# proger/haloop

Measured on AMD Instinct MI355X. Metric: utterances/sec, LSTM-CTC training step (fwd + CTC loss + bwd + clip + AdamW), higher is better.
Workload: dtype bf16 (dense operands rounded to bf16, 1 MFMA per product, fp32 accumulate; fp32 state, CTC, optimizer and master weights); 1 GPU; LC-2x1024: conv(80->128,k5,s4) + 2-layer LSTM H=1024 + Linear(1024->32) + CTC, 80 frames x 80 mels, vocab 32, targets 5-10 symbols, dropout 0.2; batch_per_gpu=64, global_batch=64, frames=80, mels=80, parallelism=dp1, hip_graph=False, math=bf16

## Files before the change

haloop_amd/csrc/lstm.hip:

```cpp
#include <stdlib.h>
#include <string.h>
#include "halo_common.h"
#include "halo_internal.h"
#include "tiled_image.h"
#include "lstm_persist.h"

namespace {

enum YMode { Y_NONE = 0, Y_PLAIN = 1, Y_RELU = 2, Y_DROPOUT = 3 };

typedef __bf16 bf16x8 __attribute__((ext_vector_type(8)));

template <bool X3>
struct Packed {
    static constexpr int KB = X3 ? 32 : 16;
    static constexpr int BLOCK_BYTES = X3 ? 2048 : 1024;
    __device__ static __forceinline__ void store(void *img, int tile, int nk, int i, int k, float v) {
        const int blk = k / KB, kk = k % KB;
        char *base = (char *)img + ((long)tile * (nk / KB) + blk) * BLOCK_BYTES;
        if (X3) {
            const int lane = (kk >> 3) * 16 + i, e = kk & 7;
            const __bf16 hi = (__bf16)v;
            const __bf16 lo = (__bf16)(v - (float)hi);
            reinterpret_cast<__bf16 *>(base)[lane * 8 + e] = hi;
// ... 437 lines not shown
        else if (u < a.w_units + a.s_units) pack_unit<true, 2>(u - a.w_units, a.h0, a.hp0, a.H, a.B, a.H, a.h_rm, a.c0, a.c_rm);
        else if (u < a.w_units + a.s_units + a.zero_units) reinterpret_cast<uint4 *>(a.zero)[u - a.w_units - a.s_units] = make_uint4(0u, 0u, 0u, 0u);
        else reinterpret_cast<uint4 *>(a.zero2)[u - a.w_units - a.s_units - a.zero_units] = make_uint4(0u, 0u, 0u, 0u);
    }
}

struct ImageJobs {
    struct { const float *src; int R, K, ld, KT, tr, first; char *img; } job[4];
    int n, blocks, with_lo;
};
__device__ __forceinline__ void image_jobs_block(const ImageJobs &a, int b, float *tile) {
    int j = 0;
#pragma unroll
    for (int i = 1; i < 4; ++i)
        if (i < a.n && b >= a.job[i].first) j = i;
    const int local = b - a.job[j].first, kt = local % a.job[j].KT, rt = local / a.job[j].KT;
    if (a.job[j].tr)
        halo_img::prep_transposed_block(a.job[j].src, a.job[j].R, a.job[j].K, a.job[j].ld, a.job[j].img, a.job[j].KT, a.with_lo, kt, rt,
                                        reinterpret_cast<float (*)[halo_img::TR + 1]>(tile));
    else
        halo_img::prep_rowmajor_block(a.job[j].src, a.job[j].R, a.job[j].K, a.job[j].ld, a.job[j].img, a.job[j].KT, a.with_lo, kt, rt);
}
inline void image_jobs_add(ImageJobs &a, const float *src, int R, int K, int ld, int tr, char *img) {
    const int KT = (K + 31) / 32;
    a.job[a.n++] = {src, R, K, ld, KT, tr, a.blocks, img};
    a.blocks += ((R + 127) / 128) * KT;
}

struct Prologue2Args {
    const float *w[3]; void *wdst[3]; long w_units; int wK;
    const float *h0[2]; void *hp0[2]; float *h_rm[2]; const float *c0[2]; float *c_rm[2]; long s_units;
    unsigned *zero; long zero_units;
    unsigned *zero2; long zero2_units;
    char *arm[3]; int narm; long arm_units;
    int H, B;
    ImageJobs img;
};
__device__ __forceinline__ void arm_unit(const Prologue2Args &a, long v) {
    const int m = (int)(v / a.arm_units);
    const long w = v - m * a.arm_units;
    *reinterpret_cast<uint4 *>(a.arm[m] + (w >> 6) * 2048 + (w & 63) * 16) = make_uint4(~0u, ~0u, ~0u, ~0u);
}
template <int WMODE>
__global__ __launch_bounds__(256) void persist2_prologue_kernel(const Prologue2Args a) {
    if ((int)blockIdx.x < a.img.blocks) {
        __shared__ float tile[32 * (halo_img::TR + 1)];
        image_jobs_block(a.img, blockIdx.x, tile);
        return;
    }
    const long nw = 3 * a.w_units, ns = 2 * a.s_units, na = (long)a.narm * a.arm_units;
    const long total = nw + ns + a.zero_units + a.zero2_units + na;
    for (long u = (blockIdx.x - a.img.blocks) * 256L + threadIdx.x; u < total; u += (long)(gridDim.x - a.img.blocks) * 256) {
        if (u >= total - na) {
            arm_unit(a, u - (total - na));
        } else if (u < nw) {
            const int m = (int)(u / a.w_units);
            pack_unit<true, WMODE, true>(u - m * a.w_units, a.w[m], a.wdst[m], a.H, a.B, a.wK, nullptr, nullptr, nullptr);
        } else if (u < nw + ns) {
            const int l = (int)((u - nw) / a.s_units);
            pack_unit<true, 2, true>(u - nw - l * a.s_units, a.h0[l], a.hp0[l], a.H, a.B, a.H, a.h_rm[l], a.c0[l], a.c_rm[l]);
        } else if (u < nw + ns + a.zero_units) {
            reinterpret_cast<uint4 *>(a.zero)[u - nw - ns] = make_uint4(0u, 0u, 0u, 0u);
        } else {
            reinterpret_cast<uint4 *>(a.zero2)[u - nw - ns - a.zero_units] = make_uint4(0u, 0u, 0u, 0u);
        }
    }
}
// ... 788 lines not shown
        if (images_by_pack)
            HALO_TRY(halo_gemm_bf16x3_tiled(img_in, img_w, T * B, 4 * H, in_dim, l0.gates, 4 * H, b_ih[0], b_hh[0], 0, nullptr, st));
        ctx.packF_stamp = lo == 0 ? ctx.lstm_weights_stamp : 0;
        ctx.packF_reserve = reserve;
        for (int m = 0; m < 3; ++m) ctx.packF_w[m] = pa.w[m];
        memcpy(ctx.packF_dims, dims, sizeof(dims));
    }
    Persist2Fwd a;
    a.wp0 = (const char *)wp0; a.wp1 = (const char *)wp1; a.wpi = (const char *)wpi;
    a.hp0 = (char *)l0.hp; a.hp1 = (char *)l1.hp;
    a.xp = xp;
    a.gates0 = l0.gates; a.h0 = l0.h; a.c0 = l0.c;
    a.gates1 = l1.gates; a.h1 = l1.h; a.c1 = l1.c;
    a.b_ih1 = b_ih[1]; a.b_hh1 = b_hh[1];
    a.ydrop = p_drop > 0.f ? l0.ydrop : nullptr;
    a.y = y; a.y_stride_t = y_stride_t; a.y_stride_b = y_stride_b; a.y_mode = y ? (y_relu ? 2 : 1) : 0;
    a.drop = make_dropout(p_drop, seed, HALO_STREAM_LSTM_LAYER0 + (uint32_t)lo, offset, offset_dev);
    a.img_hT0 = emit_hT0; a.img_hT1 = emit_hT1; a.img_xT1 = emit_xT1;
    a.flags = flags;
    a.stamps = halo_lstm_persist_stamp_buffer();
    a.T = T; a.B = B; a.H = H;
    chain_begin(st);
    HALO_TRY(halo_lstm_persist2_fwd(a, st));
    chain_end(st, 0, 1, "lstm_persist2_fwd_kernel");
    for (int l = 0; l < 2; ++l) {
        const LayerBufs lb = l ? l1 : l0;
        if (hn) HALO_TRY(copy_d2d(hn + (size_t)(lo + l) * BH, lb.h + (size_t)T * BH, BH, st));
        if (cn) HALO_TRY(copy_d2d(cn + (size_t)(lo + l) * BH, lb.c + (size_t)T * BH, BH, st));
    }
    return HALO_OK;
}


inline size_t bwd_p2_offset(int T, int B, int in0, int H, int L) {
    const size_t n = bwd_flags_offset(T, B, in0, H, L) + PERSIST_FLAG_BYTES + (size_t)((B + 15) / 16) * 4 * H * sizeof(float);
    return (n + 255) & ~(size_t)255;
}
inline size_t bwd_p2_bytes(int T, int B, int H) {
    return (((size_t)((B + 15) / 16) * 4 * H * sizeof(float) + 255) & ~(size_t)255) + (size_t)T * bt16(B) * 4 * H * sizeof(float) +
           halo_tiled_image_bytes(4 * H, T * B);
}

}

extern "C" {

int halo_lstm_chain_events(void *ev_begin, void *ev_end) {
    halo_ctx_cur().chain_ev0 = (hipEvent_t)ev_begin;
    halo_ctx_cur().chain_ev1 = (hipEvent_t)ev_end;
    return HALO_OK;
}

int halo_lstm_chain_info(int backward, int *launches, char *kernel, int kernel_len) {
    const ChainInfo &ci = g_chain_info[backward ? 1 : 0];
    if (launches) *launches = ci.launches;
    if (kernel && kernel_len > 0) {
        strncpy(kernel, ci.kernel, (size_t)kernel_len - 1);
        kernel[kernel_len - 1] = 0;
    }
    return HALO_OK;
}

size_t halo_lstm_reserve_bytes(int T, int B, int in0, int H, int L) {
    if (T <= 0 || B <= 0 || in0 <= 0 || H <= 0 || L <= 0) return 0;
    return reserve_flags_offset(T, B, in0, H, L) + PERSIST_FLAG_BYTES + (L >= 2 ? reserve_p2_bytes(T, B, in0, H) : 0);
}
// ... 210 lines not shown
    char *img_g = img_gT + halo_tiled_image_bytes(4 * H, T * B);
    char *img_hT = img_g + halo_tiled_image_bytes(T * B, 4 * H);
    char *img_inT = img_hT + halo_tiled_image_bytes(kin, T * B);
    char *img_wT = img_inT + halo_tiled_image_bytes(kin, T * B);
    const bool fused = fused_ok(H, L);
    if (fused && layer_end == L) {
        float *extra = (float *)(img_wT + halo_tiled_image_bytes(kin, 4 * H));
        HALO_TRY(lstm_bwd_fused_chain(w_ih, w_hh, dy, y_stride_t, y_stride_b, y_relu, dhn, dcn, reserve, extra, T, B, H, L,
                                      p_drop, seed, offset, offset_dev, st));
    }
    int top_end = layer_end;
    if (!fused && x3 && L >= 2 && layer_begin <= L - 2 && layer_end == L && halo_lstm_persist2_ok(T, B, H, L)) {
        const int lo = L - 2, hi = L - 1;
        for (int l = lo; l <= hi; ++l) HALO_CHECK_ARG(w_ih[l] && w_hh[l] && dw_ih[l] && dw_hh[l] && db_ih[l] && db_hh[l]);
        const LayerBufs l0 = layer_bufs(reserve, lo, T, B, H), l1 = layer_bufs(reserve, hi, T, B, H);
        const float *in_lo = lo == 0 ? x : (p_drop > 0.f ? layer_bufs(reserve, lo - 1, T, B, H).ydrop : layer_bufs(reserve, lo - 1, T, B, H).h + BH);
        const int in_lo_dim = lo == 0 ? in0 : H;
        float *extra = (float *)(img_wT + halo_tiled_image_bytes(kin, 4 * H));
        float *wpT0 = wpT, *wpT1 = extra, *wpTi = extra + (size_t)4 * H * H, *dcarry1 = extra + (size_t)8 * H * H;
        char *flag_base = (char *)workspace + bwd_flags_offset(T, B, in0, H, L);
        float *bias_part0 = (float *)(flag_base + PERSIST_FLAG_BYTES);
        char *p2 = (char *)workspace + bwd_p2_offset(T, B, in0, H, L);
        float *bias_part1 = (float *)p2;
        float *dgp1 = (float *)(p2 + (((size_t)((B + 15) / 16) * 4 * H * sizeof(float) + 255) & ~(size_t)255));
        char *img_gT1 = (char *)(dgp1 + (size_t)T * PG);
        const bool can_emit = persist_emit_enabled() && B % 32 == 0;
        const bool emit0 = can_emit && in_lo_dim >= 64, emit1 = can_emit;
        const bool need_din = lo > 0 || dx != nullptr;
        float *din_out = lo > 0 ? din : dx;
        HaloCtx &ctx = halo_ctx_cur();
        const bool have_T = ctx.packT_reserve == reserve && ctx.packT_w[0] == w_hh[lo] && ctx.packT_w[1] == w_hh[hi] && ctx.packT_w[2] == w_ih[hi];
        const bool clean = have_T && ctx.bwdflags_reserve == reserve;
        ctx.bwdflags_reserve = nullptr;
        if (clean) flag_base = (char *)reserve_bwd_flags(reserve, T, B, in0, H, L);
        if (have_T) {
            float *wT = (float *)((char *)reserve + reserve_flags_offset(T, B, in0, H, L) + PERSIST_FLAG_BYTES);
            wpT0 = wT; wpT1 = wT + (size_t)4 * H * H; wpTi = wT + (size_t)8 * H * H;
        }
        Prologue2Args pa;
        pa.img.n = 0; pa.img.blocks = 0; pa.img.with_lo = 0;
        pa.w[0] = w_hh[lo]; pa.wdst[0] = wpT0; pa.w[1] = w_hh[hi]; pa.wdst[1] = wpT1; pa.w[2] = w_ih[hi]; pa.wdst[2] = wpTi;
        pa.w_units = have_T ? 0 : (long)(H / 16) * (4 * H / 32) * 64; pa.wK = 4 * H;
        for (int l = 0; l < 2; ++l) { pa.h0[l] = nullptr; pa.hp0[l] = nullptr; pa.h_rm[l] = nullptr; pa.c0[l] = nullptr; pa.c_rm[l] = nullptr; }
        pa.s_units = 0;
        pa.zero = (unsigned *)flag_base; pa.zero_units = (long)(PERSIST_FLAG_BYTES / 16);
        pa.zero2 = nullptr; pa.zero2_units = 0;
        pa.narm = 0; pa.arm_units = 0;
        if (emit0 && need_din && (T * B) % 128 != 0) {
            const long tile_bytes = (long)(4 * H / 32) * 16384;
            pa.zero2 = (unsigned *)(img_g + (long)((T * B) / 128) * tile_bytes); pa.zero2_units = tile_bytes / 16;
        }
        pa.H = H; pa.B = B;
        if (!clean) {
            hipLaunchKernelGGL(persist2_prologue_kernel<1>, dim3(pack_grid((size_t)(3 * pa.w_units + pa.zero_units + pa.zero2_units))), dim3(256), 0,
                               st, pa);
            HALO_TRY(halo_launch_status());
        }
        Persist2Bwd a;
        a.wpT0 = (const char *)wpT0; a.wpT1 = (const char *)wpT1; a.wpTi = (const char *)wpTi;
        a.dgp0 = (char *)dgp; a.dgp1 = (char *)dgp1;
        a.gates0 = l0.gates; a.gates1 = l1.gates; a.c0 = l0.c; a.c1 = l1.c;
        a.dc0 = dcarry; a.dc1 = dcarry1;
        a.dy = dy; a.dy_stride_t = y_stride_t; a.dy_stride_b = y_stride_b; a.dy_relu = y_relu;
        a.dhinit0 = dhn ? dhn + (size_t)lo * BH : nullptr; a.dcinit0 = dcn ? dcn + (size_t)lo * BH : nullptr;
        a.dhinit1 = dhn ? dhn + (size_t)hi * BH : nullptr; a.dcinit1 = dcn ? dcn + (size_t)hi * BH : nullptr;
        a.drop = make_dropout(p_drop, seed, HALO_STREAM_LSTM_LAYER0 + (uint32_t)lo, offset, offset_dev);
        a.flags = (unsigned *)flag_base;
        a.abort_word = (unsigned *)((char *)workspace + bwd_flags_offset(T, B, in0, H, L));
        a.stamps = halo_lstm_persist_stamp_buffer();
        a.img_rows0 = emit0 && need_din ? img_g : nullptr;
        a.img_cols0 = emit0 ? img_gT : nullptr;
        a.img_cols1 = emit1 ? img_gT1 : nullptr;
        a.bias_part0 = emit0 ? bias_part0 : nullptr;
        a.bias_part1 = emit1 ? bias_part1 : nullptr;
        a.skip_dg0 = !keep_dg_switch() && emit0 && (!need_din || a.img_rows0);
        a.skip_dg1 = !keep_dg_switch() && emit1;
        a.T = T; a.B = B; a.H = H;
        chain_begin(st);
        HALO_TRY(halo_lstm_persist2_bwd(a, st));
        chain_end(st, 1, 1, "lstm_persist2_bwd_kernel");
        if (ctx.emitT_reserve == reserve && emit0 && emit1 && pair_dw_enabled()) {
            char *imgs = reserve_p2_images(reserve, T, B, in0, H, L);
            const size_t hb = halo_tiled_image_bytes(H, T * B), ib = halo_tiled_image_bytes(kin, T * B);
            char *hT0 = imgs, *inT0 = imgs + hb, *hT1 = imgs + hb + ib;
            HaloPrepJob jobs[4];
            int nj = 0;
            for (int l = 1; l >= 0; --l) {
                HaloSmallJob j = {};
// ... 159 lines not shown
```

haloop_amd/csrc/lstm_persist.h:

```cpp
#pragma once
#include <hip/hip_runtime.h>
#include "halo_common.h"

constexpr int PERSIST_FLAG_HEADER = 16;
constexpr int PERSIST_MAX_BLOCKS = 256;
constexpr int PERSIST_REPLICAS = 8;
constexpr int PERSIST_REPLICA_WORDS = 1024;
constexpr size_t PERSIST_FLAG_BYTES = (size_t)PERSIST_REPLICAS * PERSIST_REPLICA_WORDS * sizeof(unsigned);

struct PersistFwd {
    const char *wp;
    char *hp;
    float *gates;
    float *h;
    float *c;
    float *y;
    long y_stride_t, y_stride_b;
    int y_mode;
    DropoutCfg drop;
    unsigned *flags;
    unsigned *status;
    int mute;
    unsigned long long *stamps;
    int poll_mode;
// ... 48 lines not shown
    unsigned *flags;
    unsigned *status;
    int mute;
    unsigned long long *stamps;
    int poll_mode, replica_shift, nap;
    int T, B, H;
    int bt0, nbt;
    unsigned epoch0;
};

struct Persist2Bwd {
    const char *wpT0, *wpT1, *wpTi;
    char *dgp0, *dgp1;
    float *gates0, *gates1;
    const float *c0, *c1;
    float *dc0, *dc1;
    const float *dy;
    long dy_stride_t, dy_stride_b;
    int dy_relu;
    const float *dhinit0, *dcinit0, *dhinit1, *dcinit1;
    DropoutCfg drop;
    unsigned *flags;
    unsigned *abort_word;
   
    unsigned *status;
    unsigned long long *stamps;
    char *img_rows0, *img_cols0, *img_cols1;
    float *bias_part0, *bias_part1;
    int skip_dg0, skip_dg1;
    int poll_mode, replica_shift, nap;
    int T, B, H;
    int bt0, nbt;
    unsigned epoch0;
};

bool halo_lstm_persist2_ok(int T, int B, int H, int L);
bool halo_lstm_persist2_dataflag();
bool halo_lstm_persist2_fwd_armed(int T, int B, int H);
void halo_lstm_persist2_enable(int on);
void halo_lstm_interleave_enable(int on);
int halo_lstm_persist2_fwd(const Persist2Fwd &a, hipStream_t st);
int halo_lstm_persist2_bwd(const Persist2Bwd &a, hipStream_t st);
int halo_lstm_persist2x_fwd(const Persist2Fwd &a, hipStream_t st);
int halo_lstm_persist2x_bwd(const Persist2Bwd &a, hipStream_t st);
```

haloop_amd/csrc/lstm_persist2.hip:

```cpp
#include <stdlib.h>
#include "halo_common.h"
#include "halo_internal.h"
#include "lstm_persist.h"
#include "lstm_persist_dev.h"

namespace {

__device__ __forceinline__ bf16x8 unarm(bf16x8 v) {
    u32x4 w = __builtin_bit_cast(u32x4, v);
    if ((w.x & 0xffffu) == 0xffffu) w.x -= 1u;
    return __builtin_bit_cast(bf16x8, w);
}
template <int N>
__device__ __forceinline__ bool armed_lane(const bf16x8 (&f)[N]) {
    bool a = false;
#pragma unroll
    for (int i = 0; i < N; ++i) a |= (__builtin_bit_cast(u32x4, f[i]).x & 0xffffu) == 0xffffu;
    return a;
}
__device__ __forceinline__ bool rearm_wait(unsigned long long &t0, int pass, int nap) {
    const unsigned long long now = __builtin_amdgcn_s_memrealtime();
    if (pass == 0) t0 = now;
    else if (now - t0 > SPIN_TIMEOUT_TICKS) return false;
    if (nap == 1) __builtin_amdgcn_s_sleep(1);
    else if (nap == 2) __builtin_amdgcn_s_sleep(4);
    else if (nap == 3) __builtin_amdgcn_s_sleep(16);
    return true;
}
__device__ __forceinline__ void stamp_value(unsigned long long *stamps, int T, int step, int point, int lane, unsigned v) {
    if (stamps && lane == 0) stamps[((long)blockIdx.x * T + step) * 16 + point] = v;
}

struct Fwd2Shared {
    float (*red)[4][4][256];
    float (*hbuf)[16][16];
    int *s_abort;
    unsigned *s_published;
};

template <int KBQ, bool DF>
__device__ __forceinline__ void fwd2_layer0_waves(const Persist2Fwd &p, const Fwd2Shared sh, int jt, int bt, int wave, int lane, int u) {
    const int wq = wave & 3;
    const int H = p.H, B = p.B, T = p.T;
    const int NJ = H / 16, NBT = (B + 15) / 16, nkb = H / 32, j0 = jt * 16;
    bf16x8 wr[4][KBQ];
#pragma unroll
    for (int g = 0; g < 4; ++g)
#pragma unroll
        for (int i = 0; i < KBQ; ++i)
            wr[g][i] = *reinterpret_cast<const bf16x8 *>(p.wp0 + (((long)jt * 4 + g) * nkb + wq * KBQ + i) * 2048 + lane * 16);
    const int ci = u >> 4, cj = u & 15;
    const int b = bt * 16 + ci;
    const bool cell = b < B;
    const int BH = B * H;
    const int e0 = b * H + j0 + cj;
    float cst = 0.f, gin[4] = {0.f, 0.f, 0.f, 0.f};
    float dmul = (cell && p.xp) ? dropout_mult(p.drop, (uint64_t)e0) : 1.f;
    if (cell) {
        cst = p.c0[e0];
// ... 281 lines not shown

template <int KBQ, bool DF>
__global__ __launch_bounds__(512, 2) void lstm_persist2_fwd_kernel(const Persist2Fwd p) {
    __shared__ float red[2][4][4][256];
    __shared__ __attribute__((aligned(16))) float hbuf[3][16][16];
    __shared__ int s_abort;
    __shared__ unsigned s_published;
    extern __shared__ __attribute__((aligned(16))) char wi_lds[];
    const int tid = threadIdx.x, lane = tid & 63;
    const int wave = __builtin_amdgcn_readfirstlane(tid >> 6);
    int jt, bt;
    map_block(blockIdx.x, gridDim.x, p.H / 16, p.nbt, jt, bt);
    bt += p.bt0;
    if (tid == 0) { s_abort = 0; s_published = 0; }
    if (wave == 0) stamp(p.stamps, p.T + 2, 0, 14, lane);
    const Fwd2Shared sh = {red, hbuf, &s_abort, &s_published};
    if (wave < 4) fwd2_layer0_waves<KBQ, DF>(p, sh, jt, bt, wave, lane, tid & 255);
    else fwd2_layer1_waves<KBQ, DF>(p, sh, wi_lds, jt, bt, wave, lane, tid & 255);
    if (wave == 0) stamp(p.stamps, p.T + 2, 0, 15, lane);
}

struct Bwd2Shared {
    float (*red)[4][256];
    float (*dgbuf)[4][16][16];
    int *s_abort;
    unsigned *s_published;
};

struct Bwd2Cell {
    float gv[4], cc, cprev, dcarry;
    __device__ __forceinline__ void update(float dh, float (&dg)[4]) { dcarry = persist2_bwd_cell(gv, cc, cprev, dcarry, dh, dg); }
};

template <int KC>
__device__ __forceinline__ void bwd2_layer0_waves(const Persist2Bwd &p, const Bwd2Shared sh, int jt, int bt, int wave, int lane, int u) {
    constexpr int KBW = 4 * KC, CH = 4, NCH = KBW / CH, NBUF = 3;
    const int wq = wave & 3;
    const int H = p.H, B = p.B, T = p.T, K = 4 * H;
    const int NJ = H / 16, NBT = (B + 15) / 16, nkb4 = K / 32, j0 = jt * 16;
    bf16x8 wr[KBW];
#pragma unroll
    for (int i = 0; i < KBW; ++i) wr[i] = *reinterpret_cast<const bf16x8 *>(p.wpT0 + ((long)jt * nkb4 + wq * KBW + i) * 2048 + lane * 16);
    const int ci = u >> 4, cj = u & 15;
    const int b = bt * 16 + ci;
    const bool cell = b < B;
    const int BH = B * H;
    const int e0 = b * H + j0 + cj;
    Bwd2Cell c;
    c.cc = c.cprev = c.dcarry = 0.f;
    float dh0 = 0.f, bsum[4] = {0.f, 0.f, 0.f, 0.f};
    float dmul = cell ? dropout_mult(p.drop, (uint64_t)((long)(T - 1) * BH + e0)) : 1.f;
#pragma unroll
    for (int g = 0; g < 4; ++g) c.gv[g] = 0.f;
    if (cell) {
        const int t = T - 1;
#pragma unroll
        for (int g = 0; g < 4; ++g) c.gv[g] = p.gates0[(t * B + b) * K + g * H + j0 + cj];
        c.cc = p.c0[(t + 1) * BH + e0];
        c.cprev = p.c0[t * BH + e0];
        if (p.dcinit0) c.dcarry = p.dcinit0[e0];
        if (p.dhinit0) dh0 = p.dhinit0[e0];
    }
    const __amdgpu_buffer_rsrc_t dg0_rsrc = make_rsrc(p.dgp0), dg1_rsrc = make_rsrc(p.dgp1);
    const int my_replica = (xcc_id() + p.replica_shift) % PERSIST_REPLICAS;
    const int btl = bt - p.bt0;
    const unsigned *grp_flags = p.flags + my_replica * PERSIST_REPLICA_WORDS + PERSIST_FLAG_HEADER + btl * NJ;
    for (int s = 0; s <= T; ++s) {
        if (wave == 0) stamp(p.stamps, T + 1, s, 0, lane);
        const bool act = s >= 1;
        const int t = T - s;
        bool ok = true;
        if (s > 0 && wave == 1) ok = poll_group(grp_flags, 0, NJ, p.epoch0 + (unsigned)s, lane, p.nap);
        if (!ok && lane == 0) {
            *sh.s_abort = 1;
            raise_abort(p.abort_word, p.status);
        }
        lds_barrier();
        if (*sh.s_abort) return;
        if (wave == 0) stamp(p.stamps, T + 1, s, 1, lane);
        f32x4 acc = {0.f, 0.f, 0.f, 0.f};
        if (s >= 2) {
            const int img = (((T - s + 1) * NBT + bt) * nkb4 + wq * KBW) * 2048;
            bf16x8 ah[NBUF][CH];
            auto loadc = [&](int buf, int cidx) {
#pragma unroll
                for (int i = 0; i < CH; ++i) ah[buf][i] = load_sc1_u(dg0_rsrc, lane * 16, img + (cidx * CH + i) * 2048);
            };
#pragma unroll
            for (int cidx = 0; cidx < NBUF - 1 && cidx < NCH; ++cidx) loadc(cidx, cidx);
#pragma unroll
            for (int cidx = 0; cidx < NCH; ++cidx) {
                if (cidx + NBUF - 1 < NCH) loadc((cidx + NBUF - 1) % NBUF, cidx + NBUF - 1);
                __builtin_amdgcn_sched_barrier(0);
#pragma unroll
                for (int i = 0; i < CH; ++i) acc = __builtin_amdgcn_mfma_f32_16x16x32_bf16(ah[cidx % NBUF][i], wr[cidx * CH + i], acc, 0, 0, 0);
            }
        }
        {
            const int r = lane & 15, q = lane >> 4;
#pragma unroll
            for (int e = 0; e < 4; ++e) sh.red[0][wq][(4 * q + e) * 16 + r] = acc[e];
        }
        lds_barrier();
        if (wave == 0) stamp(p.stamps, T + 1, s, 2, lane);
        float dg[4] = {0.f, 0.f, 0.f, 0.f};
        if (act) {
            if (cell) {
                float rec = 0.f, above = 0.f;
#pragma unroll
                for (int k = 0; k < 4; ++k) { rec += sh.red[0][k][u]; above += sh.red[2][k][u]; }
                c.update(persist2_add_masked(s == 1 ? dh0 : rec, above, dmul), dg);
#pragma unroll
                for (int g = 0; g < 4; ++g) bsum[g] += dg[g];
            }
#pragma unroll
            for (int g = 0; g < 4; ++g) sh.dgbuf[0][g][ci][cj] = dg[g];
        }
        lds_barrier();
        if (wave == 0) stamp(p.stamps, T + 1, s, 3, lane);
        {
            const int g = wq, lay = lane < 32 ? 1 : 0, kg = (lane >> 4) & 1, row = lane & 15;
            const bool on = lay ? (s < T) : (s >= 1);
            const int tt = lay ? T - 1 - s : T - s;
            bf16x8 hi;
            if (on) {
#pragma unroll
                for (int e = 0; e < 8; ++e) hi[e] = (__bf16)sh.dgbuf[lay][g][row][kg * 8 + e];
                const int dst = ((tt * NBT + bt) * nkb4 + g * (H / 32) + (jt >> 1)) * 2048 + (((jt & 1) * 2 + kg) * 16 + row) * 16;
                if (lay) store_sc1(dg1_rsrc, dst, hi);
                else store_sc1(dg0_rsrc, dst, hi);
            }
            asm volatile("s_waitcnt vmcnt(0)" ::: "memory");
            unsigned old = 0;
            if (lane == 0) old = atomicAdd(sh.s_published, 1u);
            old = __builtin_amdgcn_readfirstlane(old);
            if (old == 4u * (unsigned)s + 3u) publish_epoch(p.flags, btl * NJ + jt, p.epoch0 + (unsigned)(s + 1), lane);
            if (wave == 3) stamp(p.stamps, T + 1, s, 4, lane);
            if (on) {
                char *img_rows = lay ? nullptr : p.img_rows0;
                char *img_cols = lay ? p.img_cols1 : p.img_cols0;
                if (img_rows) {
                    const int grow = tt * B + bt * 16 + row, kcol = g * H + j0 + kg * 8;
                    const long blk = ((long)(grow >> 7) * nkb4 + (kcol >> 5)) * 2;
                    const int r = grow & 127, cc = (kcol & 31) >> 3;
                    *reinterpret_cast<bf16x8 *>(img_rows + blk * 8192 + r * 64 + ((cc ^ ((r >> 2) & 3)) << 4)) = hi;
                }
                if (img_cols) {
                    bf16x8 hit;
#pragma unroll
                    for (int e = 0; e < 8; ++e) hit[e] = (__bf16)sh.dgbuf[lay][g][kg * 8 + e][row];
                    const int grow = g * H + j0 + row, kcol = tt * B + bt * 16 + kg * 8;
                    const int KT = (T * B + 31) >> 5;
                    const long blk = ((long)(grow >> 7) * KT + (kcol >> 5)) * 2;
                    const int r = grow & 127, cc = (kcol & 31) >> 3;
                    *reinterpret_cast<bf16x8 *>(img_cols + blk * 8192 + r * 64 + ((cc ^ ((r >> 2) & 3)) << 4)) = hit;
                }
            }
        }
        if (act && cell) {
            float *gp = p.gates0 + (t * B + b) * K + j0 + cj;
            if (!p.skip_dg0) { gp[0] = dg[0]; gp[H] = dg[1]; gp[2 * H] = dg[2]; gp[3 * H] = dg[3]; }
            if (t > 0) {
                dmul = dropout_mult(p.drop, (uint64_t)((long)(t - 1) * BH + e0));
#pragma unroll
                for (int g = 0; g < 4; ++g) c.gv[g] = p.gates0[((t - 1) * B + b) * K + g * H + j0 + cj];
                c.cc = c.cprev;
                c.cprev = p.c0[(t - 1) * BH + e0];
            }
        }
    }
    if (cell && p.dc0) p.dc0[e0] = c.dcarry;
    lds_barrier();
#pragma unroll
    for (int g = 0; g < 4; ++g) sh.dgbuf[0][g][ci][cj] = bsum[g];
    lds_barrier();
    if (p.bias_part0 && u < 64) {
        const int g = u >> 4, j = u & 15;
        float sum = 0.f;
#pragma unroll
        for (int r = 0; r < 16; ++r) sum += sh.dgbuf[0][g][r][j];
        p.bias_part0[(long)bt * K + g * H + j0 + j] = sum;
    }
}

template <int KC>
__device__ __forceinline__ void bwd2_layer1_waves(const Persist2Bwd &p, const Bwd2Shared sh, char *wi_lds, int jt, int bt, int wave, int lane,
                                                  int u) {
    constexpr int KBW = 4 * KC, CH = 4, NCH = KBW / CH, NBUF = 3;
    const int wq = wave & 3;
    const int H = p.H, B = p.B, T = p.T, K = 4 * H;
    const int NBT = (B + 15) / 16, nkb4 = K / 32, j0 = jt * 16;
    bf16x8 wr[KBW];
#pragma unroll
    for (int i = 0; i < KBW; ++i) wr[i] = *reinterpret_cast<const bf16x8 *>(p.wpT1 + ((long)jt * nkb4 + wq * KBW + i) * 2048 + lane * 16);
    char *my_wi = wi_lds + (long)wq * KBW * 1024 + lane * 16;
#pragma unroll
    for (int i = 0; i < KBW; ++i) {
        *reinterpret_cast<bf16x8 *>(my_wi + i * 1024) =
            *reinterpret_cast<const bf16x8 *>(p.wpTi + ((long)jt * nkb4 + wq * KBW + i) * 2048 + lane * 16);
        if ((i & 15) == 15) __builtin_amdgcn_sched_barrier(0);
    }
    const int ci = u >> 4, cj = u & 15;
    const int b = bt * 16 + ci;
    const bool cell = b < B;
    const int BH = B * H;
    const int e0 = b * H + j0 + cj;
    Bwd2Cell c;
    c.cc = c.cprev = c.dcarry = 0.f;
    float dh0 = 0.f, dyv = 0.f, bsum[4] = {0.f, 0.f, 0.f, 0.f};
#pragma unroll
    for (int g = 0; g < 4; ++g) c.gv[g] = 0.f;
    if (cell) {
        const int t = T - 1;
#pragma unroll
        for (int g = 0; g < 4; ++g) c.gv[g] = p.gates1[(t * B + b) * K + g * H + j0 + cj];
        c.cc = p.c1[(t + 1) * BH + e0];
        c.cprev = p.c1[t * BH + e0];
        if (p.dy) dyv = p.dy[(long)t * p.dy_stride_t + (long)b * p.dy_stride_b + j0 + cj];
        if (p.dcinit1) c.dcarry = p.dcinit1[e0];
        if (p.dhinit1) dh0 = p.dhinit1[e0];
    }
    const __amdgpu_buffer_rsrc_t dg1_rsrc = make_rsrc(p.dgp1);
    for (int s = 0; s <= T; ++s) {
        const bool act = s < T;
        const int t = T - 1 - s;
        lds_barrier();
        if (*sh.s_abort) return;
        f32x4 acc = {0.f, 0.f, 0.f, 0.f}, acc2 = {0.f, 0.f, 0.f, 0.f};
        if (s >= 1) {
            const int img = (((T - s) * NBT + bt) * nkb4 + wq * KBW) * 2048;
            bf16x8 ah[NBUF][CH];
            auto loadc = [&](int buf, int cidx) {
#pragma unroll
                for (int i = 0; i < CH; ++i) ah[buf][i] = load_sc1_u(dg1_rsrc, lane * 16, img + (cidx * CH + i) * 2048);
            };
#pragma unroll
            for (int cidx = 0; cidx < NBUF - 1 && cidx < NCH; ++cidx) loadc(cidx, cidx);
#pragma unroll
            for (int cidx = 0; cidx < NCH; ++cidx) {
                if (cidx + NBUF - 1 < NCH) loadc((cidx + NBUF - 1) % NBUF, cidx + NBUF - 1);
                __builtin_amdgcn_sched_barrier(0);
#pragma unroll
                for (int i = 0; i < CH; ++i) {
                    const bf16x8 w = *reinterpret_cast<const bf16x8 *>(my_wi + (cidx * CH + i) * 1024);
                    acc = __builtin_amdgcn_mfma_f32_16x16x32_bf16(ah[cidx % NBUF][i], wr[cidx * CH + i], acc, 0, 0, 0);
                    acc2 = __builtin_amdgcn_mfma_f32_16x16x32_bf16(ah[cidx % NBUF][i], w, acc2, 0, 0, 0);
                }
            }
        }
        {
            const int r = lane & 15, q = lane >> 4;
#pragma unroll
            for (int e = 0; e < 4; ++e) {
                sh.red[1][wq][(4 * q + e) * 16 + r] = acc[e];
                sh.red[2][wq][(4 * q + e) * 16 + r] = acc2[e];
            }
        }
        lds_barrier();
        float dg[4] = {0.f, 0.f, 0.f, 0.f};
        if (act) {
            if (cell) {
                float dh = 0.f;
                if (s == 0) dh = dh0;
                else {
#pragma unroll
                    for (int k = 0; k < 4; ++k) dh += sh.red[1][k][u];
                }
                if (p.dy) {
                    const float tc = persist2_tanh(c.cc);
                    float d = dyv;
                    if (p.dy_relu && !(c.gv[3] * tc > 0.f)) d = 0.f;
                    dh += d;
                }
                c.update(dh, dg);
#pragma unroll
                for (int g = 0; g < 4; ++g) bsum[g] += dg[g];
            }
#pragma unroll
            for (int g = 0; g < 4; ++g) sh.dgbuf[1][g][ci][cj] = dg[g];
        }
        lds_barrier();
        if (act && cell) {
            float *gp = p.gates1 + (t * B + b) * K + j0 + cj;
            if (!p.skip_dg1) { gp[0] = dg[0]; gp[H] = dg[1]; gp[2 * H] = dg[2]; gp[3 * H] = dg[3]; }
            if (t > 0) {
#pragma unroll
                for (int g = 0; g < 4; ++g) c.gv[g] = p.gates1[((t - 1) * B + b) * K + g * H + j0 + cj];
                c.cc = c.cprev;
                c.cprev = p.c1[(t - 1) * BH + e0];
                if (p.dy) dyv = p.dy[(long)(t - 1) * p.dy_stride_t + (long)b * p.dy_stride_b + j0 + cj];
            }
        }
    }
    if (cell && p.dc1) p.dc1[e0] = c.dcarry;
    lds_barrier();
#pragma unroll
    for (int g = 0; g < 4; ++g) sh.dgbuf[1][g][ci][cj] = bsum[g];
    lds_barrier();
    if (p.bias_part1 && u < 64) {
        const int g = u >> 4, j = u & 15;
        float sum = 0.f;
#pragma unroll
        for (int r = 0; r < 16; ++r) sum += sh.dgbuf[1][g][r][j];
        p.bias_part1[(long)bt * K + g * H + j0 + j] = sum;
    }
}

template <int KC>
__global__ __launch_bounds__(512, 2) void lstm_persist2_bwd_kernel(const Persist2Bwd p) {
    __shared__ float red[3][4][256];
    __shared__ __attribute__((aligned(16))) float dgbuf[2][4][16][16];
    __shared__ int s_abort;
    __shared__ unsigned s_published;
    extern __shared__ __attribute__((aligned(16))) char wi_lds[];
    const int tid = threadIdx.x, lane = tid & 63;
    const int wave = __builtin_amdgcn_readfirstlane(tid >> 6);
    int jt, bt;
    map_block(blockIdx.x, gridDim.x, p.H / 16, p.nbt, jt, bt);
    bt += p.bt0;
    if (tid == 0) { s_abort = 0; s_published = 0; }
    if (blockIdx.x == 0 && tid == 0 && p.abort_word != p.flags) __hip_atomic_store(p.abort_word, 0u, __ATOMIC_RELAXED, __HIP_MEMORY_SCOPE_AGENT);
    if (wave == 0) stamp(p.stamps, p.T + 1, 0, 14, lane);
    const Bwd2Shared sh = {red, dgbuf, &s_abort, &s_published};
    if (wave < 4) bwd2_layer0_waves<KC>(p, sh, jt, bt, wave, lane, tid & 255);
    else bwd2_layer1_waves<KC>(p, sh, wi_lds, jt, bt, wave, lane, tid & 255);
    if (wave == 0) stamp(p.stamps, p.T + 1, 0, 15, lane);
}

int g_cu_count2 = 0;
inline int cu_count2() {
    if (!g_cu_count2) {
        int dev = 0;
        hipDeviceProp_t prop;
        if (hipGetDevice(&dev) == hipSuccess && hipGetDeviceProperties(&prop, dev) == hipSuccess) g_cu_count2 = prop.multiProcessorCount;
        else g_cu_count2 = -1;
    }
    return g_cu_count2;
}

inline int tiles_per_launch(int H) { return max(1, cu_count2() / (H / 16)); }

constexpr size_t MIN_DYN_LDS = 64 * 1024;

inline void set_mute(Persist2Fwd &a) { a.mute = halo_ctx_cur().mute_block; }
inline void set_mute(Persist2Bwd &) {}

template <typename K, typename A>
int launch2(K kernel, const A &a0, int blocks, size_t dyn, hipStream_t st) {
    static_assert(sizeof(A) <= 4096, "kernel arguments");
    A a = a0;
    static const int shift = getenv("HALO_PERSIST_REPLICA_SHIFT") ? atoi(getenv("HALO_PERSIST_REPLICA_SHIFT")) : 3;
    static const int nap = getenv("HALO_PERSIST_NAP") ? atoi(getenv("HALO_PERSIST_NAP")) : 2;
    a.poll_mode = 0; a.replica_shift = shift; a.nap = nap;
    a.status = halo_ctx_cur().status;
    set_mute(a);
    if (dyn < MIN_DYN_LDS) dyn = MIN_DYN_LDS;
    if (hipFuncSetAttribute((const void *)kernel, hipFuncAttributeMaxDynamicSharedMemorySize, (int)dyn) != hipSuccess) return HALO_ELAUNCH;
    hipLaunchKernelGGL(kernel, dim3((unsigned)blocks), dim3(512), dyn, st, a);
    return halo_launch_status();
}

}

void halo_lstm_persist2_enable(int on) { halo_ctx_cur().lstm_persistent2 = on ? 1 : 0; }
void halo_lstm_interleave_enable(int on) { halo_ctx_cur().lstm_interleave = on ? 1 : 0; }

bool halo_lstm_persist2_ok(int T, int B, int H, int L) {
    static const bool env_off = getenv("HALO_LSTM_PERSIST2") && atoi(getenv("HALO_LSTM_PERSIST2")) == 0;
    if (env_off || !halo_ctx_cur().lstm_persistent2) return false;
    if (!halo_lstm_persist_ok(16, H) || B <= 0 || !halo_lstm_persist_fits(T, B, H)) return false;
    if (halo_math_mode() != HALO_MATH_BF16 || L < 2) return false;
    if (H % 128 != 0 || H > 1024 || T < 1) return false;
    const long nbt = (B + 15) / 16;
    if ((long)(T + 2) * nbt * (4 * H / 32) * 2048 >= (1L << 31)) return false;
    if ((long)(T + 1) * B * 4 * H >= (1L << 31)) return false;
    return H / 16 <= cu_count2() && PERSIST_FLAG_HEADER + 2L * tiles_per_launch(H) * (H / 16) <= PERSIST_REPLICA_WORDS;
}

inline bool interleave_on() {
    static const bool env_off = getenv("HALO_LSTM_INTERLEAVE") && atoi(getenv("HALO_LSTM_INTERLEAVE")) == 0;
    return !env_off && halo_ctx_cur().lstm_interleave != 0;
}
inline bool pairs_for(int T, int B, int H) {
    return (B + 15) / 16 > tiles_per_launch(H) && interleave_on() && (long)(T + 1) * B * 4 * H * (long)sizeof(float) < (1L << 31);
}

bool halo_lstm_persist2_dataflag() {
    static const bool on = !(getenv("HALO_PERSIST_DATAFLAG") && atoi(getenv("HALO_PERSIST_DATAFLAG")) == 0);
    return on;
}
bool halo_lstm_persist2_fwd_armed(int T, int B, int H) { return halo_lstm_persist2_dataflag() && !pairs_for(T, B, H); }

template <typename A, typename F, typename FX>
int launch_groups(const A &a0, int steps, F launch_one, FX launch_pairs) {
    const int nbt = (a0.B + 15) / 16, per = tiles_per_launch(a0.H);
    const bool pairs = pairs_for(a0.T, a0.B, a0.H);
    for (int bt0 = 0, g = 0; bt0 < nbt; ++g) {
        A a = a0;
        const int left = nbt - bt0;
        a.bt0 = bt0; a.epoch0 = (unsigned)g * (unsigned)(steps + 2);
        int rc;
        const int two = min(2 * per, left) & ~1;
        if (pairs && two > per) {
            a.nbt = two;
            rc = launch_pairs(a);
        } else {
            a.nbt = min(per, left);
            rc = launch_one(a, (a.H / 16) * a.nbt);
        }
        if (rc != HALO_OK) return rc;
        bt0 += a.nbt;
    }
    return HALO_OK;
}

int halo_lstm_persist2_fwd(const Persist2Fwd &a0, hipStream_t st) {
    const int kbq = a0.H / 128;
    const size_t dyn = (size_t)4 * 1024 * (4 * kbq - (kbq >= 8 ? 2 : 0));
    const bool df = halo_lstm_persist2_fwd_armed(a0.T, a0.B, a0.H);
    return launch_groups(a0, a0.T + 2, [&](const Persist2Fwd &a, int blocks) {
        switch (kbq * 2 + (df ? 1 : 0)) {
            case 4: return launch2(lstm_persist2_fwd_kernel<2, false>, a, blocks, dyn, st);
            case 5: return launch2(lstm_persist2_fwd_kernel<2, true>, a, blocks, dyn, st);
            case 8: return launch2(lstm_persist2_fwd_kernel<4, false>, a, blocks, dyn, st);
            case 9: return launch2(lstm_persist2_fwd_kernel<4, true>, a, blocks, dyn, st);
            case 12: return launch2(lstm_persist2_fwd_kernel<6, false>, a, blocks, dyn, st);
            case 13: return launch2(lstm_persist2_fwd_kernel<6, true>, a, blocks, dyn, st);
            case 16: return launch2(lstm_persist2_fwd_kernel<8, false>, a, blocks, dyn, st);
            case 17: return launch2(lstm_persist2_fwd_kernel<8, true>, a, blocks, dyn, st);
            default: return (int)HALO_ENOTSUP;
        }
    }, [&](const Persist2Fwd &a) { return halo_lstm_persist2x_fwd(a, st); });
}

int halo_lstm_persist2_bwd(const Persist2Bwd &a0, hipStream_t st) {
    const int kc = a0.H / 128;
    const size_t dyn = (size_t)4 * 4 * kc * 1024;
    return launch_groups(a0, a0.T + 1, [&](const Persist2Bwd &a, int blocks) {
        switch (kc) {
            case 2: return launch2(lstm_persist2_bwd_kernel<2>, a, blocks, dyn, st);
            case 4: return launch2(lstm_persist2_bwd_kernel<4>, a, blocks, dyn, st);
            case 6: return launch2(lstm_persist2_bwd_kernel<6>, a, blocks, dyn, st);
            case 8: return launch2(lstm_persist2_bwd_kernel<8>, a, blocks, dyn, st);
            default: return (int)HALO_ENOTSUP;
        }
    }, [&](const Persist2Bwd &a) { return halo_lstm_persist2x_bwd(a, st); });
}
```

Baseline: 155,200 utterances/s.

## Use data-as-flag armed images for persistent LSTM backward instead of epoch flags

Extends the data-flag synchronization already used in the forward persistent kernel to the backward kernel. The prologue fills the dgate images with a sentinel bit pattern, consumers spin on the loaded data until no lane holds the sentinel, and producers store unarmed values and no longer wait on vmcnt or publish epoch flags. Loads of the next step's gates and cell state are prefetched through buffer loads while the current step is still in flight. The intent is to remove the flag round-trip and the store-drain wait from the per-timestep critical path, at the cost of an extra prologue arming pass on every call and more spinning on the data buffers themselves.

Result: no change. 155,800 utterances/s (median of 6 runs) (+0.4%).

```diff
diff --git a/haloop_amd/csrc/lstm.hip b/haloop_amd/csrc/lstm.hip
--- a/haloop_amd/csrc/lstm.hip
+++ b/haloop_amd/csrc/lstm.hip
@@ -493,7 +493,7 @@
     const float *h0[2]; void *hp0[2]; float *h_rm[2]; const float *c0[2]; float *c_rm[2]; long s_units;
     unsigned *zero; long zero_units;
     unsigned *zero2; long zero2_units;
-    char *arm[3]; int narm; long arm_units;
+    char *arm[8]; int narm; long arm_units;
     int H, B;
     ImageJobs img;
 };
@@ -1348,6 +1348,12 @@
 }
 
 
+inline void arm_bwd_images(Prologue2Args &pa, char *dg0, char *dg1, int T, int B, int H) {
+    const long blocks = (long)T * ((B + 15) / 16) * (H / 32);
+    pa.arm_units = blocks * 64;
+    for (int m = 0; m < 8; ++m) pa.arm[pa.narm++] = (m < 4 ? dg0 : dg1) + (m & 3) * blocks * 2048;
+}
+
 inline size_t bwd_p2_offset(int T, int B, int in0, int H, int L) {
     const size_t n = bwd_flags_offset(T, B, in0, H, L) + PERSIST_FLAG_BYTES + (size_t)((B + 15) / 16) * 4 * H * sizeof(float);
     return (n + 255) & ~(size_t)255;
@@ -1624,6 +1630,7 @@
         const bool have_T = ctx.packT_reserve == reserve && ctx.packT_w[0] == w_hh[lo] && ctx.packT_w[1] == w_hh[hi] && ctx.packT_w[2] == w_ih[hi];
         const bool clean = have_T && ctx.bwdflags_reserve == reserve;
         ctx.bwdflags_reserve = nullptr;
+        const bool arm = halo_lstm_persist2_bwd_armed(T, B, H);
         if (clean) flag_base = (char *)reserve_bwd_flags(reserve, T, B, in0, H, L);
         if (have_T) {
             float *wT = (float *)((char *)reserve + reserve_flags_offset(T, B, in0, H, L) + PERSIST_FLAG_BYTES);
@@ -1642,10 +1649,11 @@
             const long tile_bytes = (long)(4 * H / 32) * 16384;
             pa.zero2 = (unsigned *)(img_g + (long)((T * B) / 128) * tile_bytes); pa.zero2_units = tile_bytes / 16;
         }
+        if (arm) arm_bwd_images(pa, (char *)dgp, (char *)dgp1, T, B, H);
         pa.H = H; pa.B = B;
-        if (!clean) {
-            hipLaunchKernelGGL(persist2_prologue_kernel<1>, dim3(pack_grid((size_t)(3 * pa.w_units + pa.zero_units + pa.zero2_units))), dim3(256), 0,
-                               st, pa);
+        if (!clean || arm) {
+            hipLaunchKernelGGL(persist2_prologue_kernel<1>, dim3(pack_grid((size_t)(3 * pa.w_units + pa.zero_units + pa.zero2_units +
+                                                                                     (long)pa.narm * pa.arm_units))), dim3(256), 0, st, pa);
             HALO_TRY(halo_launch_status());
         }
         Persist2Bwd a;
diff --git a/haloop_amd/csrc/lstm_persist.h b/haloop_amd/csrc/lstm_persist.h
--- a/haloop_amd/csrc/lstm_persist.h
+++ b/haloop_amd/csrc/lstm_persist.h
@@ -104,11 +104,13 @@
     int T, B, H;
     int bt0, nbt;
     unsigned epoch0;
+    int mute;
 };
 
 bool halo_lstm_persist2_ok(int T, int B, int H, int L);
 bool halo_lstm_persist2_dataflag();
 bool halo_lstm_persist2_fwd_armed(int T, int B, int H);
+bool halo_lstm_persist2_bwd_armed(int T, int B, int H);
 void halo_lstm_persist2_enable(int on);
 void halo_lstm_interleave_enable(int on);
 int halo_lstm_persist2_fwd(const Persist2Fwd &a, hipStream_t st);
diff --git a/haloop_amd/csrc/lstm_persist2.hip b/haloop_amd/csrc/lstm_persist2.hip
--- a/haloop_amd/csrc/lstm_persist2.hip
+++ b/haloop_amd/csrc/lstm_persist2.hip
@@ -25,6 +25,21 @@
     if (nap == 1) __builtin_amdgcn_s_sleep(1);
     else if (nap == 2) __builtin_amdgcn_s_sleep(4);
     else if (nap == 3) __builtin_amdgcn_s_sleep(16);
+    return true;
+}
+template <int N, typename R>
+__device__ __forceinline__ bool settle(const bf16x8 (&f)[N], R reload, unsigned long long &t0, unsigned &reloads, int nap) {
+    if (!__any(armed_lane<N>(f))) return true;
+    do {
+        const unsigned long long now = __builtin_amdgcn_s_memrealtime();
+        if (reloads == 0) t0 = now;
+        else if (now - t0 > SPIN_TIMEOUT_TICKS) return false;
+        ++reloads;
+        if (nap == 1) __builtin_amdgcn_s_sleep(1);
+        else if (nap == 2) __builtin_amdgcn_s_sleep(4);
+        else if (nap == 3) __builtin_amdgcn_s_sleep(16);
+        reload();
+    } while (__any(armed_lane<N>(f)));
     return true;
 }
 __device__ __forceinline__ void stamp_value(unsigned long long *stamps, int T, int step, int point, int lane, unsigned v) {
@@ -372,7 +387,7 @@
     __device__ __forceinline__ void update(float dh, float (&dg)[4]) { dcarry = persist2_bwd_cell(gv, cc, cprev, dcarry, dh, dg); }
 };
 
-template <int KC>
+template <int KC, bool DF>
 __device__ __forceinline__ void bwd2_layer0_waves(const Persist2Bwd &p, const Bwd2Shared sh, int jt, int bt, int wave, int lane, int u) {
     constexpr int KBW = 4 * KC, CH = 4, NCH = KBW / CH, NBUF = 3;
     const int wq = wave & 3;
@@ -389,18 +404,37 @@
     Bwd2Cell c;
     c.cc = c.cprev = c.dcarry = 0.f;
     float dh0 = 0.f, bsum[4] = {0.f, 0.f, 0.f, 0.f};
-    float dmul = cell ? dropout_mult(p.drop, (uint64_t)((long)(T - 1) * BH + e0)) : 1.f;
+    float dmul = 1.f;
+    DropoutCfg drop = p.drop;
 #pragma unroll
     for (int g = 0; g < 4; ++g) c.gv[g] = 0.f;
-    if (cell) {
-        const int t = T - 1;
-#pragma unroll
-        for (int g = 0; g < 4; ++g) c.gv[g] = p.gates0[(t * B + b) * K + g * H + j0 + cj];
-        c.cc = p.c0[(t + 1) * BH + e0];
-        c.cprev = p.c0[t * BH + e0];
-        if (p.dcinit0) c.dcarry = p.dcinit0[e0];
-        if (p.dhinit0) dh0 = p.dhinit0[e0];
-    }
+    if constexpr (DF) {
+        if (drop.offset_dev) { drop.offset += *drop.offset_dev; drop.offset_dev = nullptr; }
+        if (cell) {
+            if (p.dcinit0) c.dcarry = p.dcinit0[e0];
+            if (p.dhinit0) dh0 = p.dhinit0[e0];
+        }
+    } else {
+        dmul = cell ? dropout_mult(p.drop, (uint64_t)((long)(T - 1) * BH + e0)) : 1.f;
+        if (cell) {
+            const int t = T - 1;
+#pragma unroll
+            for (int g = 0; g < 4; ++g) c.gv[g] = p.gates0[(t * B + b) * K + g * H + j0 + cj];
+            c.cc = p.c0[(t + 1) * BH + e0];
+            c.cprev = p.c0[t * BH + e0];
+            if (p.dcinit0) c.dcarry = p.dcinit0[e0];
+            if (p.dhinit0) dh0 = p.dhinit0[e0];
+        }
+    }
+    const __amdgpu_buffer_rsrc_t g0_rsrc = make_rsrc(p.gates0), c0_rsrc = make_rsrc(p.c0);
+    const int vg = ((min(b, B - 1) * K) + j0 + cj) * 4, vc = (min(b, B - 1) * H + j0 + cj) * 4;
+    auto prefetch = [&](int ns) {
+        const int tn = min(max(T - ns, 0), T - 1);
+#pragma unroll
+        for (int g = 0; g < 4; ++g) c.gv[g] = load_f32_u(g0_rsrc, vg, (tn * B * K + g * H) * 4);
+        c.cc = load_f32_u(c0_rsrc, vc, (tn + 1) * BH * 4);
+        c.cprev = load_f32_u(c0_rsrc, vc, tn * BH * 4);
+    };
     const __amdgpu_buffer_rsrc_t dg0_rsrc = make_rsrc(p.dgp0), dg1_rsrc = make_rsrc(p.dgp1);
     const int my_replica = (xcc_id() + p.replica_shift) % PERSIST_REPLICAS;
     const int btl = bt - p.bt0;
@@ -409,17 +443,48 @@
         if (wave == 0) stamp(p.stamps, T + 1, s, 0, lane);
         const bool act = s >= 1;
         const int t = T - s;
-        bool ok = true;
-        if (s > 0 && wave == 1) ok = poll_group(grp_flags, 0, NJ, p.epoch0 + (unsigned)s, lane, p.nap);
-        if (!ok && lane == 0) {
-            *sh.s_abort = 1;
-            raise_abort(p.abort_word, p.status);
+        if constexpr (!DF) {
+            bool ok = true;
+            if (s > 0 && wave == 1) ok = poll_group(grp_flags, 0, NJ, p.epoch0 + (unsigned)s, lane, p.nap);
+            if (!ok && lane == 0) {
+                *sh.s_abort = 1;
+                raise_abort(p.abort_word, p.status);
+            }
         }
         lds_barrier();
         if (*sh.s_abort) return;
         if (wave == 0) stamp(p.stamps, T + 1, s, 1, lane);
         f32x4 acc = {0.f, 0.f, 0.f, 0.f};
-        if (s >= 2) {
+        if constexpr (DF) {
+            const bool use = s >= 2;
+            const int img = ((min(T - s + 1, T - 1) * NBT + bt) * nkb4 + wq * KBW) * 2048;
+            bf16x8 ah[NBUF][CH];
+            auto loadc = [&](int buf, int cidx) {
+#pragma unroll
+                for (int i = 0; i < CH; ++i) ah[buf][i] = load_sc1_u(dg0_rsrc, lane * 16, img + (cidx * CH + i) * 2048);
+            };
+#pragma unroll
+            for (int cidx = 0; cidx < NBUF - 1 && cidx < NCH; ++cidx) loadc(cidx, cidx);
+            __builtin_amdgcn_sched_barrier(0);
+            if (act && cell) dmul = dropout_mult(drop, (uint64_t)((long)t * BH + e0));
+            __builtin_amdgcn_sched_barrier(0);
+            unsigned long long t0 = 0;
+            unsigned reloads = 0;
+            bool live = true;
+#pragma unroll
+            for (int cidx = 0; cidx < NCH; ++cidx) {
+                if (cidx + NBUF - 1 < NCH) loadc((cidx + NBUF - 1) % NBUF, cidx + NBUF - 1);
+                __builtin_amdgcn_sched_barrier(0);
+                if (use && live && !settle<CH>(ah[cidx % NBUF], [&] { loadc(cidx % NBUF, cidx); }, t0, reloads, p.nap)) {
+                    live = false;
+                    if (lane == 0) { *sh.s_abort = 1; raise_abort(p.abort_word, p.status); }
+                }
+#pragma unroll
+                for (int i = 0; i < CH; ++i) acc = __builtin_amdgcn_mfma_f32_16x16x32_bf16(ah[cidx % NBUF][i], wr[cidx * CH + i], acc, 0, 0, 0);
+            }
+            if (!use) acc = f32x4{0.f, 0.f, 0.f, 0.f};
+            if (wave == 0) { stamp(p.stamps, T + 1, s, 10, lane); stamp_value(p.stamps, T + 1, s, 11, lane, reloads); }
+        } else if (s >= 2) {
             const int img = (((T - s + 1) * NBT + bt) * nkb4 + wq * KBW) * 2048;
             bf16x8 ah[NBUF][CH];
             auto loadc = [&](int buf, int cidx) {
@@ -442,6 +507,7 @@
             for (int e = 0; e < 4; ++e) sh.red[0][wq][(4 * q + e) * 16 + r] = acc[e];
         }
         lds_barrier();
+        if (DF && *sh.s_abort) return;
         if (wave == 0) stamp(p.stamps, T + 1, s, 2, lane);
         float dg[4] = {0.f, 0.f, 0.f, 0.f};
         if (act) {
@@ -456,6 +522,7 @@
 #pragma unroll
             for (int g = 0; g < 4; ++g) sh.dgbuf[0][g][ci][cj] = dg[g];
         }
+        if (DF) prefetch(s + 1);
         lds_barrier();
         if (wave == 0) stamp(p.stamps, T + 1, s, 3, lane);
         {
@@ -467,14 +534,23 @@
 #pragma unroll
                 for (int e = 0; e < 8; ++e) hi[e] = (__bf16)sh.dgbuf[lay][g][row][kg * 8 + e];
                 const int dst = ((tt * NBT + bt) * nkb4 + g * (H / 32) + (jt >> 1)) * 2048 + (((jt & 1) * 2 + kg) * 16 + row) * 16;
-                if (lay) store_sc1(dg1_rsrc, dst, hi);
-                else store_sc1(dg0_rsrc, dst, hi);
-            }
-            asm volatile("s_waitcnt vmcnt(0)" ::: "memory");
-            unsigned old = 0;
-            if (lane == 0) old = atomicAdd(sh.s_published, 1u);
-            old = __builtin_amdgcn_readfirstlane(old);
-            if (old == 4u * (unsigned)s + 3u) publish_epoch(p.flags, btl * NJ + jt, p.epoch0 + (unsigned)(s + 1), lane);
+                if constexpr (DF) {
+                    if ((int)blockIdx.x != p.mute) {
+                        if (lay) store_sc1(dg1_rsrc, dst, unarm(hi));
+                        else store_sc1(dg0_rsrc, dst, unarm(hi));
+                    }
+                } else {
+                    if (lay) store_sc1(dg1_rsrc, dst, hi);
+                    else store_sc1(dg0_rsrc, dst, hi);
+                }
+            }
+            if constexpr (!DF) {
+                asm volatile("s_waitcnt vmcnt(0)" ::: "memory");
+                unsigned old = 0;
+                if (lane == 0) old = atomicAdd(sh.s_published, 1u);
+                old = __builtin_amdgcn_readfirstlane(old);
+                if (old == 4u * (unsigned)s + 3u) publish_epoch(p.flags, btl * NJ + jt, p.epoch0 + (unsigned)(s + 1), lane);
+            }
             if (wave == 3) stamp(p.stamps, T + 1, s, 4, lane);
             if (on) {
                 char *img_rows = lay ? nullptr : p.img_rows0;
@@ -500,7 +576,7 @@
         if (act && cell) {
             float *gp = p.gates0 + (t * B + b) * K + j0 + cj;
             if (!p.skip_dg0) { gp[0] = dg[0]; gp[H] = dg[1]; gp[2 * H] = dg[2]; gp[3 * H] = dg[3]; }
-            if (t > 0) {
+            if (!DF && t > 0) {
                 dmul = dropout_mult(p.drop, (uint64_t)((long)(t - 1) * BH + e0));
 #pragma unroll
                 for (int g = 0; g < 4; ++g) c.gv[g] = p.gates0[((t - 1) * B + b) * K + g * H + j0 + cj];
@@ -523,7 +599,7 @@
     }
 }
 
-template <int KC>
+template <int KC, bool DF>
 __device__ __forceinline__ void bwd2_layer1_waves(const Persist2Bwd &p, const Bwd2Shared sh, char *wi_lds, int jt, int bt, int wave, int lane,
                                                   int u) {
     constexpr int KBW = 4 * KC, CH = 4, NCH = KBW / CH, NBUF = 3;
@@ -550,7 +626,25 @@
     float dh0 = 0.f, dyv = 0.f, bsum[4] = {0.f, 0.f, 0.f, 0.f};
 #pragma unroll
     for (int g = 0; g < 4; ++g) c.gv[g] = 0.f;
-    if (cell) {
+    const __amdgpu_buffer_rsrc_t g1_rsrc = make_rsrc(p.gates1), c1_rsrc = make_rsrc(p.c1);
+    const int vg = ((min(b, B - 1) * K) + j0 + cj) * 4, vc = (min(b, B - 1) * H + j0 + cj) * 4;
+    const float *dyp = p.dy ? p.dy : p.c1;
+    const long vdy = p.dy ? (long)min(b, B - 1) * p.dy_stride_b + j0 + cj : 0L, dy_t = p.dy ? p.dy_stride_t : 0L;
+    auto prefetch = [&](int ns) {
+        const int tn = min(max(T - 1 - ns, 0), T - 1);
+#pragma unroll
+        for (int g = 0; g < 4; ++g) c.gv[g] = load_f32_u(g1_rsrc, vg, (tn * B * K + g * H) * 4);
+        c.cc = load_f32_u(c1_rsrc, vc, (tn + 1) * BH * 4);
+        c.cprev = load_f32_u(c1_rsrc, vc, tn * BH * 4);
+        dyv = dyp[vdy + (long)tn * dy_t];
+    };
+    if constexpr (DF) {
+        prefetch(0);
+        if (cell) {
+            if (p.dcinit1) c.dcarry = p.dcinit1[e0];
+            if (p.dhinit1) dh0 = p.dhinit1[e0];
+        }
+    } else if (cell) {
         const int t = T - 1;
 #pragma unroll
         for (int g = 0; g < 4; ++g) c.gv[g] = p.gates1[(t * B + b) * K + g * H + j0 + cj];
@@ -567,8 +661,9 @@
         lds_barrier();
         if (*sh.s_abort) return;
         f32x4 acc = {0.f, 0.f, 0.f, 0.f}, acc2 = {0.f, 0.f, 0.f, 0.f};
-        if (s >= 1) {
-            const int img = (((T - s) * NBT + bt) * nkb4 + wq * KBW) * 2048;
+        if constexpr (DF) {
+            const bool use = s >= 1;
+            const int img = ((min(T - s, T - 1) * NBT + bt) * nkb4 + wq * KBW) * 2048;
             bf16x8 ah[NBUF][CH];
             auto loadc = [&](int buf, int cidx) {
 #pragma unroll
@@ -576,10 +671,17 @@
             };
 #pragma unroll
             for (int cidx = 0; cidx < NBUF - 1 && cidx < NCH; ++cidx) loadc(cidx, cidx);
+            unsigned long long t0 = 0;
+            unsigned reloads = 0;
+            bool live = true;
 #pragma unroll
             for (int cidx = 0; cidx < NCH; ++cidx) {
                 if (cidx + NBUF - 1 < NCH) loadc((cidx + NBUF - 1) % NBUF, cidx + NBUF - 1);
                 __builtin_amdgcn_sched_barrier(0);
+                if (use && live && !settle<CH>(ah[cidx % NBUF], [&] { loadc(cidx % NBUF, cidx); }, t0, reloads, p.nap)) {
+                    live = false;
+                    if (lane == 0) { *sh.s_abort = 1; raise_abort(p.abort_word, p.status); }
+                }
 #pragma unroll
                 for (int i = 0; i < CH; ++i) {
                     const bf16x8 w = *reinterpret_cast<const bf16x8 *>(my_wi + (cidx * CH + i) * 1024);
@@ -587,6 +689,28 @@
                     acc2 = __builtin_amdgcn_mfma_f32_16x16x32_bf16(ah[cidx % NBUF][i], w, acc2, 0, 0, 0);
                 }
             }
+            if (!use) { acc = f32x4{0.f, 0.f, 0.f, 0.f}; acc2 = f32x4{0.f, 0.f, 0.f, 0.f}; }
+            if (wave == 4) { stamp(p.stamps, T + 1, s, 12, lane); stamp_value(p.stamps, T + 1, s, 13, lane, reloads); }
+        } else if (s >= 1) {
+            const int img = (((T - s) * NBT + bt) * nkb4 + wq * KBW) * 2048;
+            bf16x8 ah[NBUF][CH];
+            auto loadc = [&](int buf, int cidx) {
+#pragma unroll
+                for (int i = 0; i < CH; ++i) ah[buf][i] = load_sc1_u(dg1_rsrc, lane * 16, img + (cidx * CH + i) * 2048);
+            };
+#pragma unroll
+            for (int cidx = 0; cidx < NBUF - 1 && cidx < NCH; ++cidx) loadc(cidx, cidx);
+#pragma unroll
+            for (int cidx = 0; cidx < NCH; ++cidx) {
+                if (cidx + NBUF - 1 < NCH) loadc((cidx + NBUF - 1) % NBUF, cidx + NBUF - 1);
+                __builtin_amdgcn_sched_barrier(0);
+#pragma unroll
+                for (int i = 0; i < CH; ++i) {
+                    const bf16x8 w = *reinterpret_cast<const bf16x8 *>(my_wi + (cidx * CH + i) * 1024);
+                    acc = __builtin_amdgcn_mfma_f32_16x16x32_bf16(ah[cidx % NBUF][i], wr[cidx * CH + i], acc, 0, 0, 0);
+                    acc2 = __builtin_amdgcn_mfma_f32_16x16x32_bf16(ah[cidx % NBUF][i], w, acc2, 0, 0, 0);
+                }
+            }
         }
         {
             const int r = lane & 15, q = lane >> 4;
@@ -597,6 +721,7 @@
             }
         }
         lds_barrier();
+        if (DF && *sh.s_abort) return;
         float dg[4] = {0.f, 0.f, 0.f, 0.f};
         if (act) {
             if (cell) {
@@ -619,11 +744,12 @@
 #pragma unroll
             for (int g = 0; g < 4; ++g) sh.dgbuf[1][g][ci][cj] = dg[g];
         }
+        if (DF) prefetch(s + 1);
         lds_barrier();
         if (act && cell) {
             float *gp = p.gates1 + (t * B + b) * K + j0 + cj;
             if (!p.skip_dg1) { gp[0] = dg[0]; gp[H] = dg[1]; gp[2 * H] = dg[2]; gp[3 * H] = dg[3]; }
-            if (t > 0) {
+            if (!DF && t > 0) {
 #pragma unroll
                 for (int g = 0; g < 4; ++g) c.gv[g] = p.gates1[((t - 1) * B + b) * K + g * H + j0 + cj];
                 c.cc = c.cprev;
@@ -646,7 +772,7 @@
     }
 }
 
-template <int KC>
+template <int KC, bool DF>
 __global__ __launch_bounds__(512, 2) void lstm_persist2_bwd_kernel(const Persist2Bwd p) {
     __shared__ float red[3][4][256];
     __shared__ __attribute__((aligned(16))) float dgbuf[2][4][16][16];
@@ -662,8 +788,8 @@
     if (blockIdx.x == 0 && tid == 0 && p.abort_word != p.flags) __hip_atomic_store(p.abort_word, 0u, __ATOMIC_RELAXED, __HIP_MEMORY_SCOPE_AGENT);
     if (wave == 0) stamp(p.stamps, p.T + 1, 0, 14, lane);
     const Bwd2Shared sh = {red, dgbuf, &s_abort, &s_published};
-    if (wave < 4) bwd2_layer0_waves<KC>(p, sh, jt, bt, wave, lane, tid & 255);
-    else bwd2_layer1_waves<KC>(p, sh, wi_lds, jt, bt, wave, lane, tid & 255);
+    if (wave < 4) bwd2_layer0_waves<KC, DF>(p, sh, jt, bt, wave, lane, tid & 255);
+    else bwd2_layer1_waves<KC, DF>(p, sh, wi_lds, jt, bt, wave, lane, tid & 255);
     if (wave == 0) stamp(p.stamps, p.T + 1, 0, 15, lane);
 }
 
@@ -683,7 +809,7 @@
 constexpr size_t MIN_DYN_LDS = 64 * 1024;
 
 inline void set_mute(Persist2Fwd &a) { a.mute = halo_ctx_cur().mute_block; }
-inline void set_mute(Persist2Bwd &) {}
+inline void set_mute(Persist2Bwd &a) { a.mute = halo_ctx_cur().mute_block; }
 
 template <typename K, typename A>
 int launch2(K kernel, const A &a0, int blocks, size_t dyn, hipStream_t st) {
@@ -730,6 +856,9 @@
     return on;
 }
 bool halo_lstm_persist2_fwd_armed(int T, int B, int H) { return halo_lstm_persist2_dataflag() && !pairs_for(T, B, H); }
+bool halo_lstm_persist2_bwd_armed(int T, int B, int H) {
+    return halo_lstm_persist2_fwd_armed(T, B, H) && (long)(T + 1) * B * 4 * H * (long)sizeof(float) < (1L << 31);
+}
 
 template <typename A, typename F, typename FX>
 int launch_groups(const A &a0, int steps, F launch_one, FX launch_pairs) {
@@ -776,12 +905,17 @@
 int halo_lstm_persist2_bwd(const Persist2Bwd &a0, hipStream_t st) {
     const int kc = a0.H / 128;
     const size_t dyn = (size_t)4 * 4 * kc * 1024;
+    const bool df = halo_lstm_persist2_bwd_armed(a0.T, a0.B, a0.H);
     return launch_groups(a0, a0.T + 1, [&](const Persist2Bwd &a, int blocks) {
-        switch (kc) {
-            case 2: return launch2(lstm_persist2_bwd_kernel<2>, a, blocks, dyn, st);
-            case 4: return launch2(lstm_persist2_bwd_kernel<4>, a, blocks, dyn, st);
-            case 6: return launch2(lstm_persist2_bwd_kernel<6>, a, blocks, dyn, st);
-            case 8: return launch2(lstm_persist2_bwd_kernel<8>, a, blocks, dyn, st);
+        switch (kc * 2 + (df ? 1 : 0)) {
+            case 4: return launch2(lstm_persist2_bwd_kernel<2, false>, a, blocks, dyn, st);
+            case 5: return launch2(lstm_persist2_bwd_kernel<2, true>, a, blocks, dyn, st);
+            case 8: return launch2(lstm_persist2_bwd_kernel<4, false>, a, blocks, dyn, st);
+            case 9: return launch2(lstm_persist2_bwd_kernel<4, true>, a, blocks, dyn, st);
+            case 12: return launch2(lstm_persist2_bwd_kernel<6, false>, a, blocks, dyn, st);
+            case 13: return launch2(lstm_persist2_bwd_kernel<6, true>, a, blocks, dyn, st);
+            case 16: return launch2(lstm_persist2_bwd_kernel<8, false>, a, blocks, dyn, st);
+            case 17: return launch2(lstm_persist2_bwd_kernel<8, true>, a, blocks, dyn, st);
             default: return (int)HALO_ENOTSUP;
         }
     }, [&](const Persist2Bwd &a) { return halo_lstm_persist2x_bwd(a, st); });
```
